# Orange-OpenSource/Cool-Chic

Hardware: AMD Instinct MI355X
Metric: decoded Mpixel/s (higher is better)
Workload: dtype int64+f64 entropy / f32 synthesis; 1 GPU; kodak24; frames_on_rank0=24, frame=512x768 RGB 8-bit, HOP decoder

## Files before the change

### cool_chic_amd/csrc/ccd_entropy_pipe.hip

```cpp
#include <hip/hip_runtime.h>
#include <type_traits>

#include "ccd_device.hpp"
#include "ccd_kernels.hpp"
#include "ccd_laplace.hpp"

namespace ccd {

#if defined(CCD_PIPE_PROFILE) && CCD_PIPE_PROFILE >= 3
#define PROF_T() __builtin_amdgcn_s_memtime()
#define PROF_ADD(var, t0) var += __builtin_amdgcn_s_memtime() - (t0)
#define PROF_SUB(var, t0) var -= __builtin_amdgcn_s_memtime() - (t0)
#else
#define PROF_T() 0ull
#define PROF_ADD(var, t0) (void)(t0)
#define PROF_SUB(var, t0) (void)(t0)
#endif
#if defined(CCD_PIPE_PROFILE) && CCD_PIPE_PROFILE == 2 && defined(CCD_PIPE_TRACE)
#define LPROF_T(cond) __builtin_amdgcn_s_memtime()
#elif defined(CCD_PIPE_PROFILE) && CCD_PIPE_PROFILE == 2
#define LPROF_T(cond) ((cond) ? __builtin_amdgcn_s_memtime() : 0ull)
#else
#define LPROF_T(cond) 0ull
#endif
#if defined(CCD_PIPE_TRACE)
constexpr int kTraceTasks = 512;
constexpr uint32_t kTraceLdsBytes = kTraceTasks * 32u;
__device__ unsigned int g_trace[kTraceTasks * 8];
__device__ unsigned int g_trace_cfg[2];
#endif

#ifndef CCD_T8
#define CCD_T8 25
#endif
#ifndef CCD_T4
#define CCD_T4 9
#endif
#ifndef CCD_PIPE_THREADS
#define CCD_PIPE_THREADS 512
#endif
constexpr int kPipeThreads = CCD_PIPE_THREADS;
constexpr int kPipeWaves = kPipeThreads / 64;
constexpr int kProducers = kPipeWaves - 1;
constexpr int kRows = 128;
constexpr int kSlots = 16;
constexpr int kMaxNV = 8;
constexpr int kRingRows = 512;
constexpr int kNarrowMaxScale = kScaleOffset;
constexpr int kIfceFastIn = 12;
constexpr unsigned kSpinLimit = 1u << 27;

struct alignas(16) RowMeta {
    double rcp[kRows + 2];
    int32_t mu_idx[kRows + 2];
    int32_t top[kRows + 2];
    uint32_t cell[kRows + 2];
    uint32_t goff[kRows + 2];
};
static_assert(offsetof(RowMeta, cell) - offsetof(RowMeta, top) == 520 && offsetof(RowMeta, goff) - offsetof(RowMeta, top) == 1040,
              "the decoder's asm region reads cell / goff at these immediate offsets from a top symbol's address");

extern __shared__ __attribute__((aligned(16))) unsigned char ccd_pipe_smem[];
template <typename T>
__device__ __forceinline__ T* smem_at(uint32_t off) { return reinterpret_cast<T*>(ccd_pipe_smem + off); }
template <typename T>
struct LdsRef {
    uint32_t off;
    __device__ __forceinline__ operator T*() const { return reinterpret_cast<T*>(ccd_pipe_smem + off); }
    __device__ __forceinline__ LdsRef& operator=(T* p) {
        off = static_cast<uint32_t>(reinterpret_cast<unsigned char*>(const_cast<typename std::remove_const<T>::type*>(p)) - ccd_pipe_smem);
        return *this;
    }
};

struct PipeLayout { uint32_t ring, w, b, act, a, tab, meta, rcp, exp, ready, consumed, abort, end; int n_w_hidden; };
__host__ __device__ constexpr PipeLayout pipe_layout(int dim, int n_layers, int in_pad, int ring_rows, int mf_tabs) {
    PipeLayout L{};
    L.ring = 0;
    L.w = static_cast<uint32_t>(ring_rows) * 64u;
    L.n_w_hidden = (n_layers - 1) * dim * in_pad;
    const int n_w_total = L.n_w_hidden + 4 * in_pad;
    L.b = L.w + static_cast<uint32_t>((n_w_total + 3) & ~3) * 4u;
    const int n_b_total = (n_layers - 1) * dim + 4;
    L.act = L.b + static_cast<uint32_t>((n_b_total + 1) & ~1) * 8u;
    L.a = L.act + static_cast<uint32_t>(kProducers * ((mf_tabs ? 16 : 8) * in_pad + 4)) * 4u;
    L.tab = L.a + static_cast<uint32_t>(mf_tabs) * 1024u;
    L.meta = L.tab + static_cast<uint32_t>(kRows + 1) * 64u * 8u;
    L.rcp = L.meta + static_cast<uint32_t>(sizeof(RowMeta));
    L.exp = L.rcp + static_cast<uint32_t>(kNumScale + 1) * 8u;
    L.ready = L.exp + static_cast<uint32_t>(1 << CCD_EXP_LOG) * 8u;
    L.consumed = L.ready + static_cast<uint32_t>(kSlots) * 4u;
    L.abort = L.consumed + 8u;
    L.end = (L.ready + static_cast<uint32_t>(kSlots + 8) * 4u + 15u) & ~15u;
    return L;
}

struct ShapeDyn { static constexpr bool fixed = false; static constexpr int dim = 0, n_layers = 0, n_sp = 0; };
template <int DIM, int NL, int NSP>
struct ShapeFix { static constexpr bool fixed = true; static constexpr int dim = DIM, n_layers = NL, n_sp = NSP; };
using ShapeHop = ShapeFix<20, 3, 14>;

__host__ __device__ constexpr int feat_stride(int n_if) { return n_if > 0 ? n_if : 1; }

struct PipeCtx {
    const EntropyParams* P;
    LdsRef<uint2> s_tab;
    LdsRef<RowMeta> s_meta;
    LdsRef<const double> s_rcp;
    LdsRef<const double> s_exp;
    LdsRef<int32_t> s_w;
    LdsRef<int64_t> s_b;
    LdsRef<int32_t> s_act;
    LdsRef<uint32_t> s_a;
    LdsRef<int8_t> s_ring;
    LdsRef<uint32_t> s_ready;
    LdsRef<uint32_t> s_consumed;
    LdsRef<uint32_t> s_abort;
// ... 668 lines not shown
            const uint32_t l_lo = static_cast<uint32_t>(__builtin_amdgcn_readlane(p_lo, k));
            const uint32_t l_hi = static_cast<uint32_t>(__builtin_amdgcn_readlane(p_hi, k));
            const uint32_t psel = static_cast<uint32_t>(__builtin_amdgcn_readlane(cur.y, k));
            uint64_t nd = rc_dist - ((static_cast<uint64_t>(l_hi) << 32) | l_lo);
            uint64_t nr = static_cast<uint64_t>(sc_lo) * psel + (static_cast<uint64_t>(sc_hi * psel) << 32);
            if (nr == 0) {
                S.n_search += 1;
                const uint64_t scale = rc_range >> kRcPrecision;
                if ((rc_dist >> kRcPrecision) >= scale) {
                    lds_write_release(C.s_abort, static_cast<uint32_t>(-CCD_ERR_INVALID_DATA));
                    ok = false;
                    break;
                }
                const double mu = -64.0 + static_cast<double>(meta.mu_idx[row0 + pi]) * (1.0 / 256.0);
                const double rcp = meta.rcp[row0 + pi];
                const uint32_t f0 = window_left(mu, rcp, kAcLo + lane, C.s_exp);
                const uint32_t f1 = window_left(mu, rcp, kAcLo + 64 + lane, C.s_exp);
                const unsigned long long m0 = __ballot(scale * f0 <= rc_dist), m1 = __ballot(scale * f1 <= rc_dist);
                const int sidx = __popcll(m0) + __popcll(m1) - 1;
                const uint32_t left = uni(static_cast<uint32_t>(__shfl(sidx < 64 ? f0 : f1, sidx & 63)));
                uint32_t right = uni(static_cast<uint32_t>(__shfl(sidx + 1 < 64 ? f0 : f1, (sidx + 1) & 63)));
                if (sidx == kAlphabet - 1) right = 1u << kRcPrecision;
                nd = rc_dist - scale * left;
                nr = scale * static_cast<uint64_t>(right - left);
                k = uni(1 - ((sidx + kAcLo) - meta.top[row0 + pi]));
            }
            if (static_cast<uint32_t>(nr >> 32) == 0) {
                nr <<= 32;
                nd = (nd << 32) | static_cast<uint32_t>(__builtin_amdgcn_readlane(wbuf, (word_pos - wbase) & 63));
                ++word_pos;
                if (word_pos - wbase == 64) { wbase = word_pos; wbuf = (wbase + lane < n_words) ? words_g[wbase + lane] : 0u; }
            }
            rc_dist = uni(nd); rc_range = uni(nr);
            asm volatile("s_mov_b32 m0, %2\n\tv_writelane_b32 %0, %1, m0" : "+v"(raw) : "s"(k), "s"(pi));
            ++i;
            mode = 1;
        }
    }
    S.dist = rc_dist; S.range = rc_range; S.word_pos = word_pos; S.wbase = wbase; S.wbuf = wbuf;
    S.n_spins += n_spins;
    S.n_part_batches += n_part;
    return seq;
}

__device__ __forceinline__ int64_t dot4(int4 x, int4 w) {
    return static_cast<int64_t>(x.x) * w.x + static_cast<int64_t>(x.y) * w.y + static_cast<int64_t>(x.z) * w.z +
           static_cast<int64_t>(x.w) * w.w;
}

__device__ __forceinline__ void mad64(int64_t& acc, int32_t x, int32_t w) {
    acc += static_cast<int64_t>(x) * static_cast<int64_t>(w);
    asm("" : "+v"(acc));
}
#define CCD_MAD4(ACC, X, Wv, NCH)                                                   \
    _Pragma("unroll") for (int g_ = 0; g_ < (NCH); ++g_) mad64(ACC[g_], (X).x, Wv[g_].x); \
    _Pragma("unroll") for (int g_ = 0; g_ < (NCH); ++g_) mad64(ACC[g_], (X).y, Wv[g_].y); \
    _Pragma("unroll") for (int g_ = 0; g_ < (NCH); ++g_) mad64(ACC[g_], (X).z, Wv[g_].z); \
    _Pragma("unroll") for (int g_ = 0; g_ < (NCH); ++g_) mad64(ACC[g_], (X).w, Wv[g_].w);
#define CCD_MAD4_PAIR(ACC, ACC2, X, Wv)                                             \
    mad64(ACC[0], (X).x, Wv[0].x); mad64(ACC2, (X).y, Wv[0].y); mad64(ACC[0], (X).z, Wv[0].z); mad64(ACC2, (X).w, Wv[0].w);


typedef int i32x4 __attribute__((ext_vector_type(4)));
constexpr int kMfLayer1 = 8;
constexpr int kMfHidden = 10;
constexpr int kMfOut = 5;
__host__ __device__ constexpr int mf_tables(int n_layers) { return kMfLayer1 + (n_layers - 2) * kMfHidden + kMfOut; }

__device__ __forceinline__ uint32_t mf_byte(int32_t w, int j) {
    const uint32_t d = (static_cast<uint32_t>(w) + 0x00808080u) ^ 0x00808080u;
    return (j < 0 || j > 2) ? 0u : ((d >> (8 * j)) & 0xffu);
}
__device__ __forceinline__ int mf_slot_input(bool first, int g, int beta, int n_sp, int n_if, int dim, int* limb) {
    if (first) {
        if (beta < 8) { *limb = 0; const int k = g + 4 * beta; return k < n_sp ? k : -1; }
        if (beta < 12) { *limb = (beta - 8) & 1; const int f = g + 4 * ((beta - 8) >> 1); return f < n_if ? n_sp + f : -1; }
        return -1;
    }
    if (beta >= 15) return -1;
    const int a = beta / 3;
    *limb = beta - 3 * a;
    const int k = a < 4 ? 4 * g + a : 16 + g;
    return k < dim ? k : -1;
}
__device__ __forceinline__ i32x4 mf_pack15(const int32_t (&a)[5]) {
    uint32_t d[5];
#pragma unroll
    for (int i = 0; i < 5; ++i) d[i] = ((static_cast<uint32_t>(a[i]) + 0x00808080u) ^ 0x00808080u) & 0x00ffffffu;
    i32x4 r;
    r[0] = static_cast<int>(d[0] | (d[1] << 24));
    r[1] = static_cast<int>((d[1] >> 8) | (d[2] << 16));
    r[2] = static_cast<int>((d[2] >> 16) | (d[3] << 8));
    r[3] = static_cast<int>(d[4]);
    return r;
}
__device__ __forceinline__ int64_t mf_comb4(const i32x4 (&c)[4], int r, int64_t bias) {
    const int32_t lo = c[0][r] + (c[1][r] << 8), hi = c[2][r] + (c[3][r] << 8);
    return bias + (static_cast<int64_t>(lo) << 16) + (static_cast<int64_t>(hi) << 32);
}
__device__ __forceinline__ int64_t mf_comb5(const i32x4 (&c)[5], int r, int64_t bias) {
    const int32_t lo = c[0][r] + (c[1][r] << 8), mid = c[2][r] + (c[3][r] << 8);
    return bias + lo + (static_cast<int64_t>(mid) << 16) + (static_cast<int64_t>(c[4][r]) << 32);
}

__device__ void mf_build_tables(const PipeCtx& C, int in_pad, uint32_t* s_a_words, int tid) {
    const int dim = C.dim, n_layers = C.n_layers, n_sp = C.n_sp, n_if = C.n_if;
    const int n_tab = mf_tables(n_layers);
    for (int e = tid; e < n_tab * 256; e += kPipeThreads) {
        const int idx = e >> 8, ln = (e >> 2) & 63, dw = e & 3, m = ln & 15, g = ln >> 4;
        int layer, tile, s;
        if (idx < kMfLayer1) { layer = 0; tile = idx >> 2; s = idx & 3; }
        else {
            const int j = idx - kMfLayer1, hl = j / kMfHidden;
// ... 216 lines not shown
        it.x0 = mv ? it.W - 10u : nx; it.y0 += mv; it.moved = mv; --it.left;
        it.n = min(it.H - it.y0, ((it.x0 * 0xcccdu) >> 19) + 1u);
    };
    while (n_steps_total - it.left < seg_end && it.next()) {
        const uint32_t seg_n = seg_body ? uni(seg.n_pix) : it.n;
        const uint32_t seg_pix0 = pix0;
        const uint32_t nb = (seg_n + kBpx - 1) >> kBpxShift;
        const uint32_t n_tasks = (seg_n + kTaskPix - 1) >> kTaskShift;
        const uint32_t seq0 = seq;
        uint32_t t_first = static_cast<uint32_t>(pw) - phase;
        t_first += static_cast<int32_t>(t_first) < 0 ? kProducers : 0;
        {
            for (uint32_t task = t_first; task < n_tasks; task += kProducers) {
                const uint32_t j = task >> kHalvesShift;
                const int half = static_cast<int>(task & (kHalves - 1));
                seq = seq0 + j;
                const int slot = static_cast<int>(seq & (kNSlots - 1));
                const int i0 = static_cast<int>(task << kTaskShift);
                const int cnt = min(kTaskPix, static_cast<int>(seg_n) - i0);
                while (seg_pix0 + static_cast<uint32_t>(i0) >= pix0 + it.n) walk_on();
                const uint32_t ia = seg_pix0 + static_cast<uint32_t>(i0) - pix0;
                const uint32_t n_a = min(static_cast<uint32_t>(cnt), it.n - ia);
                const uint32_t bx1 = it.x0 + 1u, b_moved = bx1 == static_cast<uint32_t>(W) ? 1u : 0u;
                const uint32_t bx0 = b_moved ? static_cast<uint32_t>(W) - 10u : bx1, by0 = it.y0 + b_moved;
                const bool in_b = static_cast<uint32_t>(px) >= n_a;
                const int ii = in_b ? px - static_cast<int>(n_a) : static_cast<int>(ia) + px;
                const int y = static_cast<int>(in_b ? by0 : it.y0) + ii, x = static_cast<int>(in_b ? bx0 : it.x0) - 10 * ii;
                const uint32_t dy1 = it.moved, dy2 = it.moved + prev_moved;
                const uint32_t prev_n = pix0 - prev_pix0, prev2_n = prev_pix0 - prev2_pix0;
                uint32_t f_raw[NOUT];
                bool f_has[NOUT];
                if constexpr (!MF) {
                    const int fo = (y >> 1) * fw + (x >> 1);
#pragma unroll
                    for (int t = 0; t < NOUT; ++t) {
                        const int k = q + kLpp * t;
                        f_has[t] = fin > 0 && px < cnt && k >= n_sp && k < dim;
                        f_raw[t] = reinterpret_cast<glb_ptr<const uint16_t>>(ifce_feat)[f_has[t] ? fo * fstride + (k - n_sp) : 0];
                    }
                } else {
#pragma unroll
                    for (int t = 0; t < NOUT; ++t) { f_raw[t] = 0; f_has[t] = false; }
                }
                unsigned long long bad_lanes = 0ull;
                const uint32_t need_slot = seq >= static_cast<uint32_t>(kNSlots) ? seq - kNSlots + 1 : 0;
                const bool ends_in_b = n_a < static_cast<uint32_t>(cnt);
                const uint32_t last1 = ends_in_b ? static_cast<uint32_t>(cnt) - n_a : ia + static_cast<uint32_t>(cnt);
                const uint32_t need_px = ends_in_b ? pix0 + min(last1 + b_moved, it.n) : prev_pix0 + min(last1 + dy1, prev_n);
                const uint32_t need_early_px = ends_in_b ? prev_pix0 + min(last1 + b_moved + dy1, prev_n)
                                                         : prev2_pix0 + min(last1 + dy2, prev2_n);
                unsigned long long lt_a = 0, lt_b = 0, lt_c = 0, lt_d = 0;
                (void)lt_a; (void)lt_b; (void)lt_c; (void)lt_d;
                unsigned narrow_mask = 0;
                unsigned long long wide_lanes = 0ull;
                RowMeta& meta = *C.s_meta;
                if constexpr (MF) {
                    const int n = px, g = q;
                    const bool live = n < cnt;
                    int32_t f0 = 0, f1 = 0;
                    if (live && fin > 0) {
                        const int fo = (y >> 1) * fw + (x >> 1);
                        if (g < n_if) f0 = ifce_feat[fo * fstride + g];
                        if (g + 4 < n_if) f1 = ifce_feat[fo * fstride + g + 4];
                    }
                    lt_a = LPROF_T(pw == 0);
#if defined(CCD_PIPE_PROFILE) && CCD_PIPE_PROFILE == 2
                    if (pw == 0 && lt_prev_end) prof[4] += lt_a - lt_prev_end;
#endif
                    {
                        const unsigned long long t0 = PROF_T();
                        if (!wait_ge2(C.s_consumed, need_slot, split ? need_early_px : need_px, C.s_abort)) return seq;
                        PROF_ADD(prof[0], t0);
                    }
                    lt_b = LPROF_T(pw == 0);
                    const unsigned long long t_g = PROF_T();
                    {
                        const int mi = (g == 0 && live) ? slot * kBpx + half * kTaskPix + n : kRows;
                        meta.cell[mi] = static_cast<uint32_t>(((y & ring_mask) << 6) | ((x + 10 * y) & 63));
                        meta.goff[mi] = static_cast<uint32_t>(y * W + x);
                    }
                    uint32_t w0 = 0, w1 = 0;
#pragma unroll
                    for (int t = 0; t < 8; ++t) {
                        if (4 * t < n_sp) {
                            const int k = g + 4 * t;
                            const int yy = y - (mf_dxy[t] >> 16), xx = x + static_cast<int16_t>(mf_dxy[t] & 0xffff);
                            const bool take = live && k < n_sp && yy >= 0 && xx >= 0 && xx < W && !(split && k == k_left);
                            const int cell = take ? (yy & ring_mask) * 64 + ((xx + 10 * yy) & 63) : 0;
                            int32_t v = C.s_ring[cell];
                            v = take ? v : 0;
                            if (t < 4) w0 |= static_cast<uint32_t>(v & 0xff) << (8 * t);
                            else w1 |= static_cast<uint32_t>(v & 0xff) << (8 * (t - 4));
                        }
                    }
                    const uint32_t d0 = (static_cast<uint32_t>(f0) + 0x8080u) ^ 0x8080u, d1 = (static_cast<uint32_t>(f1) + 0x8080u) ^ 0x8080u;
                    const i32x4 bop = {static_cast<int>(w0), static_cast<int>(w1), static_cast<int>((d0 & 0xffffu) | (d1 << 16)), 0};
                    PROF_ADD(prof[1], t_g);
                    const unsigned long long t_m = PROF_T();
                    const i32x4* sa = reinterpret_cast<const i32x4*>(static_cast<uint32_t*>(C.s_a)) + lane;
                    const i32x4 zero4 = {0, 0, 0, 0};
                    int64_t pre[5], st0, st1;
                    {
                        i32x4 c1[2][4];
#pragma unroll
                        for (int t = 0; t < 2; ++t)
#pragma unroll
// ... 180 lines not shown
#pragma unroll
                for (int v = 0; v < NV; ++v) xv[v] = act_row[v];
                PROF_ADD(prof[4], t_m);
                const unsigned long long t_s = PROF_T();
                int64_t so[2];
                const int qs = q < 2 ? q : 1;
                {
                    const int4* wr = reinterpret_cast<const int4*>(C.s_w + C.n_w_hidden + 2 * in_pad + qs * in_pad);
                    so[0] = C.s_b[(n_layers - 1) * dim + 2 + qs];
                    so[1] = 0;
                    int4 wv[NV];
#pragma unroll
                    for (int v = 0; v < NV; ++v) wv[v] = wr[v];
#pragma unroll
                    for (int v = 0; v < NV; ++v) {
                        const int4 w = wv[v];
                        mad64(so[0], xv[v].x, w.x); mad64(so[1], xv[v].y, w.y); mad64(so[0], xv[v].z, w.z); mad64(so[1], xv[v].w, w.w);
                    }
                }
                PROF_ADD(prof[5], t_s);
                const unsigned long long t_h = PROF_T();
                int64_t acc0[NOUT], acc0_b = 0;
                (void)acc0_b;
                int32_t wleft[NOUT], wleft_stab = 0;
                if (n_layers >= 2) {
                    const int32_t* wl = C.s_w;
                    const int64_t* bl = C.s_b;
                    const int4* wr[NOUT];
                    const int kl = split ? k_left : 0;
#pragma unroll
                    for (int t = 0; t < NOUT; ++t) {
                        const int oc = min(q + kLpp * t, dim - 1);
                        wr[t] = reinterpret_cast<const int4*>(wl + oc * in_pad);
                        acc0[t] = bl[oc];
                        wleft[t] = wl[oc * in_pad + kl];
                    }
                    wleft_stab = C.s_w[C.n_w_hidden + 2 * in_pad + qs * in_pad + kl];
                    int4 w[NOUT], wn[NOUT];
#pragma unroll
                    for (int t = 0; t < NOUT; ++t) w[t] = wr[t][0];
#pragma unroll
                    for (int v = 0; v < NV; ++v) {
                        if (v + 1 < NV) {
#pragma unroll
                            for (int t = 0; t < NOUT; ++t) wn[t] = wr[t][v + 1];
                        }
                        if constexpr (NOUT == 1) { CCD_MAD4_PAIR(acc0, acc0_b, xv[v], w) } else { CCD_MAD4(acc0, xv[v], w, NOUT) }
#pragma unroll
                        for (int t = 0; t < NOUT; ++t) w[t] = wn[t];
                    }
                    if constexpr (NOUT == 1) acc0[0] += acc0_b;
                }
                int32_t xleft = 0;
                lt_c = LPROF_T(pw == 0);
                if (split) {
                    const unsigned long long t0 = PROF_T();
                    const uint32_t want = uni(need_px);
                    const uint32_t cell = static_cast<uint32_t>((y & ring_mask) * 64 + ((x - 1 + 10 * y) & 63));
                    uint32_t seen_v;
                    int32_t r;
                    asm volatile("ds_read_b32 %0, %2 offset:4\n\tds_read_i8 %1, %3\n\ts_waitcnt lgkmcnt(0)"
                                 : "=&v"(seen_v), "=&v"(r) : "v"(C.s_consumed.off), "v"(C.s_ring.off + cell) : "memory");
                    if (__builtin_expect(static_cast<int32_t>(uni(seen_v) - want) < 0, 0)) {
                        unsigned spins = 0;
                        do {
                            if ((++spins & 1023u) == 0) {
                                if (lds_load_acquire(C.s_abort) != 0) return seq;
                                if (spins > kSpinLimit) { lds_write_release(C.s_abort, static_cast<uint32_t>(-CCD_ERR_HIP)); return seq; }
                            }
                            asm volatile("ds_read_b32 %0, %2 offset:4\n\tds_read_i8 %1, %3\n\ts_waitcnt lgkmcnt(0)"
                                         : "=&v"(seen_v), "=&v"(r) : "v"(C.s_consumed.off), "v"(C.s_ring.off + cell) : "memory");
                        } while (static_cast<int32_t>(uni(seen_v) - want) < 0);
                    }
                    PROF_ADD(prof[0], t0);
                    PROF_SUB(prof[2], t0);
                    PROF_SUB(prof[6], t0);
                    xleft = (px < cnt && x >= 1) ? r << 16 : 0;
                }
                lt_d = LPROF_T(pw == 0);
                __builtin_amdgcn_s_setprio(1);
                mad64(so[0], xleft, wleft_stab);
                const int64_t stab = so[0] + so[1];
                if (n_layers >= 2) {
#pragma unroll
                    for (int t = 0; t < NOUT; ++t) {
                        mad64(acc0[t], xleft, wleft[t]);
                        const int o = q + kLpp * t;
                        const int64_t a = acc0[t] < 0 ? 0 : acc0[t];
                        int32_t* const dst = o < in_pad ? act + px * in_pad + o : act_dummy;
                        *dst = o < dim ? static_cast<int32_t>(a >> 16) : 0;
                    }
#pragma unroll
                    for (int v = 0; v < NV; ++v) xv[v] = act_row[v];
                }
                for (int l = 1; l < n_layers - 1; ++l) {
                    const int32_t* wl = C.s_w + l * dim * in_pad;
                    const int64_t* bl = C.s_b + l * dim;
                    int64_t acc[NOUT], acc_b = 0;
                    (void)acc_b;
                    const int4* wr[NOUT];
#pragma unroll
                    for (int t = 0; t < NOUT; ++t) {
                        const int oc = min(q + kLpp * t, dim - 1);
                        wr[t] = reinterpret_cast<const int4*>(wl + oc * in_pad);
                        acc[t] = bl[oc];
                    }
                    int4 w[NOUT], wn[NOUT];
#pragma unroll
                    for (int t = 0; t < NOUT; ++t) w[t] = wr[t][0];
#pragma unroll
                    for (int v = 0; v < NV; ++v) {
                        if (v + 1 < NV) {
#pragma unroll
                            for (int t = 0; t < NOUT; ++t) wn[t] = wr[t][v + 1];
                        }
                        if constexpr (NOUT == 1) { CCD_MAD4_PAIR(acc, acc_b, xv[v], w) } else { CCD_MAD4(acc, xv[v], w, NOUT) }
#pragma unroll
                        for (int t = 0; t < NOUT; ++t) w[t] = wn[t];
                    }
                    if constexpr (NOUT == 1) acc[0] += acc_b;
#pragma unroll
                    for (int t = 0; t < NOUT; ++t) {
                        const int o = q + kLpp * t;
                        const int64_t a = acc[t] < 0 ? 0 : acc[t];
                        int32_t* const dst = o < in_pad ? act + px * in_pad + o : act_dummy;
                        *dst = o < dim ? static_cast<int32_t>(a >> 16) : 0;
                    }
#pragma unroll
                    for (int v = 0; v < NV; ++v) xv[v] = act_row[v];
                }
                PROF_ADD(prof[6], t_h);
                const unsigned long long t_o = PROF_T();
                const int mpx = slot * kBpx + half * kTaskPix + px;
                int32_t idx = 0;
                {
                    const int4* wr = reinterpret_cast<const int4*>(C.s_w + C.n_w_hidden + qs * in_pad);
                    int64_t ao[2] = {C.s_b[(n_layers - 1) * dim + qs] + stab, 0};
                    int4 wv[NV];
#pragma unroll
                    for (int v = 0; v < NV; ++v) wv[v] = wr[v];
#pragma unroll
                    for (int v = 0; v < NV; ++v) {
                        const int4 w = wv[v];
                        mad64(ao[0], xv[v].x, w.x); mad64(ao[1], xv[v].y, w.y); mad64(ao[0], xv[v].z, w.z); mad64(ao[1], xv[v].w, w.w);
                    }
                    const int64_t acc = ao[0] + ao[1];
                    const int64_t q8 = acc >> 24;
                    const int64_t off = q8 + (q == 0 ? kMuOffset : kScaleOffset);
                    const int64_t hi = q == 0 ? kNumMu - 1 : kNumScale - 1;
                    idx = static_cast<int32_t>(off < 0 ? 0 : (off > hi ? hi : off));
                    const bool live = px < cnt;
                    meta.mu_idx[live && q == 0 ? mpx : kRows] = idx;
                    meta.rcp[live && q == 1 ? mpx : kRows] = C.s_rcp[q == 1 ? idx : 0];
                }
                if (DYN && __builtin_expect(bad_lanes != 0ull, 0)) {
                    int n_redo = 0;
                    for (int p = 0; p < cnt; ++p) {
                        if (((bad_lanes >> (p * kLpp)) & ((1ull << kLpp) - 1ull)) == 0ull) continue;
                        ExactArgs A;
                        A.P = C.P; A.s_w = uni(C.s_w.off); A.s_b = uni(C.s_b.off); A.s_ring = uni(C.s_ring.off);
                        A.n_w_hidden = uni(C.n_w_hidden); A.dim = dim; A.n_layers = n_layers; A.n_sp = n_sp; A.in_pad = in_pad;
                        A.W = W; A.fin = fin; A.fw = fw; A.feat_plane = feat_plane; A.ring_mask = ring_mask; A.fstride = fstride;
                        asm volatile("" : "+s"(A.P), "+s"(A.s_w), "+s"(A.s_b), "+s"(A.s_ring), "+s"(A.n_w_hidden), "+s"(A.dim), "+s"(A.n_layers));
                        asm volatile("" : "+s"(A.n_sp), "+s"(A.W), "+s"(A.fin), "+s"(A.fw), "+s"(A.feat_plane), "+s"(A.ring_mask), "+s"(A.fstride));
                        const ExactOut r = exact_pixel(A, __builtin_amdgcn_readlane(y, MF ? p : p * kLpp), __builtin_amdgcn_readlane(x, MF ? p : p * kLpp));
                        if (px == p && q < 2) {
                            const int64_t off = ((q == 0 ? r.mu : r.ls) >> 24) + (q == 0 ? kMuOffset : kScaleOffset);
                            const int64_t hi = q == 0 ? kNumMu - 1 : kNumScale - 1;
                            idx = static_cast<int32_t>(off < 0 ? 0 : (off > hi ? hi : off));
                            if (q == 0) {
                                meta.mu_idx[mpx] = idx;
                            } else {
                                    meta.rcp[mpx] = C.s_rcp[idx];
                            }
                        }
                        ++n_redo;
                    }
                    if (lane == 0) atomicAdd(reinterpret_cast<int*>(P.status) + 39, n_redo);
                }
                wide_lanes = __ballot(q == 1 && px < cnt && idx > kNarrowMaxScale);
                PROF_ADD(prof[2], t_m);
                PROF_ADD(prof[7], t_o);
#if defined(CCD_PIPE_PROFILE) && CCD_PIPE_PROFILE >= 3
                prof[8] += 1;
#endif
                }
                const unsigned long long t_t = PROF_T();
                const int base = slot * kBpx + half * kTaskPix;
                uint2* tab = C.s_tab + static_cast<size_t>(base) * 64;
                if constexpr (!MF) {
                    for (int p4 = 0; p4 < cnt; p4 += 4) {
                        const int u = lane >> 4, e = lane & 15;
                        const int mine = p4 + u;
                        const bool valid = mine < cnt;
                        const int mi = base + (valid ? mine : p4);
                        const int mu_idx = meta.mu_idx[mi];
                        int top = ((mu_idx + 128) >> 8) - 64 + 6;
                        top = max(kAcLo + 13, min(kAcLo + kAlphabet - 1, top));
                        const double mu = -64.0 + static_cast<double>(mu_idx) * (1.0 / 256.0);
                        const int ssym = top - (e - 1);
                        uint32_t left = min(window_left(mu, meta.rcp[mi], ssym, C.s_exp), (1u << kRcPrecision) - 1u);
                        left = e == 15 ? 0u : left;
                        const uint32_t right = static_cast<uint32_t>(__builtin_amdgcn_update_dpp(0, static_cast<int>(left), 0x111, 0xf, 0xf, false));
                        uint2 ent;
                        ent.x = left;
                        const uint32_t to_full = (e == 1 && ssym == kAcLo + kAlphabet - 1) ? (1u << kRcPrecision) - right : 0u;
                        const uint32_t keep = (e == 0 || e == 15) ? 0u : ~0u;
                        ent.y = (right - left + to_full) & keep;
                        uint2* const row = valid ? tab + mine * 64 : C.s_tab + kRows * 64;
                        row[e] = ent;
                        meta.top[valid && e == 0 ? mi : kRows] = top;
                    }
                }
                unsigned rest = MF ? narrow_mask : 0u;
                while (rest) {
                    int pix[4];
                    int n_here = 0;
#pragma unroll
                    for (int u = 0; u < 4; ++u) {
                        pix[u] = rest ? __builtin_ctz(rest) : -1;
                        if (rest) { rest &= rest - 1; ++n_here; }
                    }
                    const int u = lane >> 4, e = lane & 15;
                    const int mine = u == 0 ? pix[0] : (u == 1 ? pix[1] : (u == 2 ? pix[2] : pix[3]));
                    const int mi = base + (mine < 0 ? pix[0] : mine);
                    const int mu_idx = meta.mu_idx[mi];
                    int top = ((mu_idx + 128) >> 8) - 64 + 6;
                    top = max(kAcLo + 13, min(kAcLo + kAlphabet - 1, top));
                    const double mu = -64.0 + static_cast<double>(mu_idx) * (1.0 / 256.0);
                    const int ssym = top - (e - 1);
                    uint32_t left = min(window_left(mu, meta.rcp[mi], ssym, C.s_exp), (1u << kRcPrecision) - 1u);
                    left = e == 15 ? 0u : left;
                    const uint32_t right = static_cast<uint32_t>(__builtin_amdgcn_update_dpp(0, static_cast<int>(left), 0x111, 0xf, 0xf, false));
                    uint2 ent;
                    ent.x = left;
                    ent.y = (e == 0 || e == 15) ? 0u : ((e == 1 && ssym == kAcLo + kAlphabet - 1) ? (1u << kRcPrecision) - left : right - left);
                    if (mine >= 0) {
                        tab[mine * 64 + e] = ent;
                        if (e == 0) meta.top[mi] = top;
                    }
                    if constexpr (MF) {
                        typedef unsigned int u32x4 __attribute__((ext_vector_type(4)));
                        const u32x4 z4 = {0u, 0u, 0u, 0u};
#pragma unroll
                        for (int j = 0; j < 2; ++j) {
                            const int t = lane + 64 * j;
                            const int ru = t >= 72 ? 3 : (t >= 48 ? 2 : (t >= 24 ? 1 : 0));
                            const int rp = ru == 0 ? pix[0] : (ru == 1 ? pix[1] : (ru == 2 ? pix[2] : pix[3]));
                            if (t < 96 && rp >= 0) *reinterpret_cast<u32x4*>(&tab[rp * 64 + 16 + 2 * (t - 24 * ru)]) = z4;
                        }
                    }
                    (void)n_here;
                }
                unsigned long long wide = MF ? static_cast<unsigned long long>(((1u << cnt) - 1u) & ~narrow_mask) : wide_lanes;
                while (wide) {
                    const int bit = __builtin_ctzll(wide);
                    wide &= wide - 1;
                    const int i = MF ? bit : bit / kLpp;
                    const int mi = base + i;
                    const int mu_idx = meta.mu_idx[mi];
                    int top = ((mu_idx + 128) >> 8) - 64 + 30;
                    top = max(kAcLo + 61, min(kAcLo + kAlphabet - 1, top));
                    const double mu = -64.0 + static_cast<double>(mu_idx) * (1.0 / 256.0);
                    const int ssym = top - (lane - 1);
                    uint32_t left = min(window_left(mu, meta.rcp[mi], ssym, C.s_exp), (1u << kRcPrecision) - 1u);
                    left = lane == 63 ? 0u : left;
                    const uint32_t right = __shfl_up(left, 1);
                    uint2 ent;
                    ent.x = left;
                    ent.y = (lane == 0 || lane == 63) ? 0u
                            : ((lane == 1 && ssym == kAcLo + kAlphabet - 1) ? (1u << kRcPrecision) - left : right - left);
                    tab[i * 64 + lane] = ent;
                    if (lane == 0) meta.top[mi] = top;
                }
                asm volatile("" ::: "memory");
                if (lane == 0) __hip_atomic_fetch_or(&C.s_ready[slot], 1u << half, __ATOMIC_RELAXED, __HIP_MEMORY_SCOPE_WORKGROUP);
                __builtin_amdgcn_s_setprio(0);
                asm volatile("" ::: "memory");
                PROF_ADD(prof[3], t_t);
#if defined(CCD_PIPE_PROFILE) && CCD_PIPE_PROFILE == 2
#if defined(CCD_PIPE_TRACE)
                {
                    const unsigned long long lt_e = __builtin_amdgcn_s_memtime();
                    const uint32_t gidx = seq0 * kHalves + task;
                    if (lane == 0 && static_cast<uint32_t>(W) == uni(g_trace_cfg[0]) && uni(g_trace_cfg[1]) - it.left < 64u) {
                        typedef unsigned int u32x4 __attribute__((ext_vector_type(4)));
                                                u32x4* r = reinterpret_cast<u32x4*>(ccd_pipe_smem + C.trace_off + (gidx % kTraceTasks) * 32u);
                        const u32x4 r0 = {(it.left << 12) | ((task & 15u) << 8) | (static_cast<uint32_t>(pw) << 4) | static_cast<uint32_t>(cnt), static_cast<uint32_t>(lt_a),
                                          static_cast<uint32_t>(lt_b), static_cast<uint32_t>(lt_c)};
                        const u32x4 r1 = {static_cast<uint32_t>(lt_d), static_cast<uint32_t>(lt_e), need_px - pix0, static_cast<uint32_t>(lt_a >> 32)};
                        r[0] = r0; r[1] = r1;
                    }
                }
#endif
                if (pw == 0) {
                    const unsigned long long lt_e = __builtin_amdgcn_s_memtime();
                    prof[0] += lt_b - lt_a; prof[1] += lt_c - lt_b; prof[2] += lt_d - lt_c; prof[3] += lt_e - lt_d; prof[8] += 1;
                    lt_prev_end = lt_e;
                }
#endif
            }
        }
        seq = seq0 + nb;
        phase = (phase + nb * kHalves) % kProducers;
        if (seg_body) {
            while (n_steps_total - it.left < seg_end) walk_on();
        }
        prev2_pix0 = prev_pix0;
        prev_pix0 = pix0;
        pix0 += it.n;
        prev_moved = it.moved;
    }
    return seq;
}

template <int NV, bool MF, bool DYN, class SH>
__global__ __launch_bounds__(kPipeThreads) void entropy_pipe_kernel(const EntropyParams* slots_desc) {
    const EntropyParams& P = slots_desc[blockIdx.x];
// ... 284 lines not shown
    }
#ifdef CCD_PIPE_PROFILE
    if (lane == 0 && wave < 2) {
        unsigned long long* o = reinterpret_cast<unsigned long long*>(P.status + 4) + wave * 5;
        o[0] = __builtin_amdgcn_s_memtime() - prof_total0;
        if (wave == 0) {
            o[1] = S.prof_wait; o[2] = S.prof_work; o[3] = prof_ifce; o[4] = prof_bar;
            P.status[38] = static_cast<int32_t>(S.n_spins);
        }
        else {
            o[1] = prof[0]; o[2] = prof[1]; o[3] = prof[2]; o[4] = prof[3];
            unsigned long long* e = reinterpret_cast<unsigned long long*>(P.status + 40);
            for (int i = 0; i < 5; ++i) e[i] = prof[4 + i];
        }
    }
#else
    (void)prof_total0; (void)prof_ifce; (void)prof_bar;
#endif
}

size_t entropy_pipe_lds_bytes(int dim, int n_layers, int ring_rows, int mfma) {
    size_t n = pipe_layout(dim, n_layers, (dim + 3) & ~3, ring_rows, mfma ? mf_tables(n_layers) : 0).end;
#if defined(CCD_PIPE_TRACE)
    n += kTraceLdsBytes;
#endif
    return n;
}

int entropy_pipe_ring_rows(int max_grid_w) {
    const int need = max_grid_w / 10 + 6;
    if (need > kRingRows) return 0;
    int r = 64;
    while (r < need) r *= 2;
    return r;
}

bool entropy_pipe_supports(int dim, int n_layers, int operands_ok, int max_grid_w) {
    const int ring = entropy_pipe_ring_rows(max_grid_w);
    return operands_ok && dim <= 4 * kMaxNV && n_layers <= 8 && ring > 0 && entropy_pipe_lds_bytes(dim, n_layers, kRingRows, 0) <= 160 * 1024;
}

bool entropy_pipe_supports_mfma(int dim, int n_layers, int n_ifce_out, int narrow, int max_grid_w, long long max_abs_weight) {
    const int ring = entropy_pipe_ring_rows(max_grid_w);
    return narrow && ring > 0 && dim <= 20 && n_layers >= 2 && n_layers <= 8 && n_ifce_out <= 8 &&
           max_abs_weight < (1ll << 23) && entropy_pipe_lds_bytes(dim, n_layers, ring, 1) <= 160 * 1024;
}

__global__ void laplace_sweep_pipe_kernel(const float* scale_table, const double* rcp_table, int scale_first, int n_scales, uint32_t* out) {
    const int64_t n = static_cast<int64_t>(n_scales) * kNumMu * 127;
    for (int64_t i = static_cast<int64_t>(blockIdx.x) * blockDim.x + threadIdx.x; i < n; i += static_cast<int64_t>(gridDim.x) * blockDim.x) {
        const int s = static_cast<int>(i % 127) - 63;
        const int64_t r = i / 127;
        const int mu_idx = static_cast<int>(r % kNumMu), c = scale_first + static_cast<int>(r / kNumMu);
        const double mu = -64.0 + static_cast<double>(mu_idx) * (1.0 / 256.0);
        out[i] = window_left(mu, rcp_table[c], s, kExpTab);
    }
}
hipError_t launch_laplace_sweep_pipe(const float* scale_table, const double* rcp_table, int scale_first, int n_scales, uint32_t* out, hipStream_t stream) {
    hipLaunchKernelGGL(laplace_sweep_pipe_kernel, dim3(256 * 16), dim3(256), 0, stream, scale_table, rcp_table, scale_first, n_scales, out);
    return hipGetLastError();
}

template <int NV, bool MF, bool DYN, class SH = ShapeDyn>
static hipError_t launch_pipe_nv(const EntropyParams* d_slots, int n_slots, size_t lds_bytes, hipStream_t stream) {
    hipError_t e = hipFuncSetAttribute(reinterpret_cast<const void*>(entropy_pipe_kernel<NV, MF, DYN, SH>),
                                       hipFuncAttributeMaxDynamicSharedMemorySize, static_cast<int>(lds_bytes));
    if (e != hipSuccess) return e;
    hipLaunchKernelGGL((entropy_pipe_kernel<NV, MF, DYN, SH>), dim3(n_slots), dim3(kPipeThreads), lds_bytes, stream, d_slots);
    return hipGetLastError();
}

int entropy_pipe_fixed_shape(int dim, int n_layers, int n_spatial) {
    return (dim == ShapeHop::dim && n_layers == ShapeHop::n_layers && n_spatial == ShapeHop::n_sp) ? 1 : 0;
}

hipError_t launch_entropy_pipe(const EntropyParams* d_slots, int n_slots, int nv, int mfma, int dyn, int shape, size_t lds_bytes, hipStream_t stream) {
    if (n_slots <= 0) return hipSuccess;
    if (shape == 1 && !mfma && nv == 5)
        return dyn ? launch_pipe_nv<5, false, true, ShapeHop>(d_slots, n_slots, lds_bytes, stream)
                   : launch_pipe_nv<5, false, false, ShapeHop>(d_slots, n_slots, lds_bytes, stream);
    if (shape != 0) return hipErrorInvalidValue;
    if (mfma) {
        switch (nv) {
            case 1: return launch_pipe_nv<1, true, false>(d_slots, n_slots, lds_bytes, stream);
            case 2: return launch_pipe_nv<2, true, false>(d_slots, n_slots, lds_bytes, stream);
            case 3: return launch_pipe_nv<3, true, false>(d_slots, n_slots, lds_bytes, stream);
            case 4: return launch_pipe_nv<4, true, false>(d_slots, n_slots, lds_bytes, stream);
            case 5: return launch_pipe_nv<5, true, false>(d_slots, n_slots, lds_bytes, stream);
            default: return hipErrorInvalidValue;
        }
    }
    if (dyn) {
        switch (nv) {
            case 1: return launch_pipe_nv<1, false, true>(d_slots, n_slots, lds_bytes, stream);
            case 2: return launch_pipe_nv<2, false, true>(d_slots, n_slots, lds_bytes, stream);
            case 3: return launch_pipe_nv<3, false, true>(d_slots, n_slots, lds_bytes, stream);
            case 4: return launch_pipe_nv<4, false, true>(d_slots, n_slots, lds_bytes, stream);
            case 5: return launch_pipe_nv<5, false, true>(d_slots, n_slots, lds_bytes, stream);
            case 6: return launch_pipe_nv<6, false, true>(d_slots, n_slots, lds_bytes, stream);
            case 7: return launch_pipe_nv<7, false, true>(d_slots, n_slots, lds_bytes, stream);
            case 8: return launch_pipe_nv<8, false, true>(d_slots, n_slots, lds_bytes, stream);
            default: return hipErrorInvalidValue;
        }
    }
    switch (nv) {
        case 1: return launch_pipe_nv<1, false, false>(d_slots, n_slots, lds_bytes, stream);
        case 2: return launch_pipe_nv<2, false, false>(d_slots, n_slots, lds_bytes, stream);
        case 3: return launch_pipe_nv<3, false, false>(d_slots, n_slots, lds_bytes, stream);
// ... 21 lines not shown
```

### cool_chic_amd/csrc/ccd_laplace.hpp

```cpp
#pragma once

#include "ccd_device.hpp"

namespace ccd {

#ifndef CCD_EXP_LOG
#define CCD_EXP_LOG 7
#endif
#ifndef CCD_EXP_DEG
#define CCD_EXP_DEG 5
#endif
#ifndef CCD_EXP_INC
#define CCD_EXP_INC "ccd_exp_table.inc"
#endif
static __device__ const double kExpTab[1 << CCD_EXP_LOG] = {
#include CCD_EXP_INC
};
constexpr int kExpLog = CCD_EXP_LOG, kExpN = 1 << kExpLog;
__device__ __forceinline__ double exp_nonpos(double x, const double* tab ) {
    const double kd = rint(x * ldexp(0x1.71547652b82fep+0, kExpLog));
    double r = fma(kd, -ldexp(0x1.62e42fef00000p-1, -kExpLog), x);
    r = fma(kd, -ldexp(0x1.473de6af278edp-34, -kExpLog), r);
    const int ki = static_cast<int>(kd);
    const double t = tab[ki & (kExpN - 1)];
    const double r2 = r * r;
#if CCD_EXP_DEG == 5
    double p = fma(r, 8.333333333333333e-03, 4.1666666666666664e-02);
    p = fma(p, r, 1.6666666666666666e-01);
    p = fma(p, r, 0.5);
#elif CCD_EXP_DEG == 4
    double p = fma(r, 4.1666666666666664e-02, 1.6666666666666666e-01);
    p = fma(p, r, 0.5);
#elif CCD_EXP_DEG == 3
    double p = fma(r, 1.6666666666666666e-01, 0.5);
#else
    double p = 0.5;
#endif
    p = fma(p, r2, r);
    return ldexp(fma(t, p, t), (ki >> kExpLog) - 1);
}

__device__ __forceinline__ uint32_t window_left(double mu, double rcp, int s, const double* exp_tab) {
    const double x = static_cast<double>(s) - 0.5;
    const double d = x - mu;
    const double e = exp_nonpos(-fabs(d) * rcp, exp_tab);
    const double cdf = d <= 0.0 ? e : 1.0 - e;
    const uint32_t v = static_cast<uint32_t>(16777088.0 * cdf) + static_cast<uint32_t>(s - kAcLo);
    return s <= kAcLo ? 0u : (s > kAcLo + kAlphabet - 1 ? (1u << kRcPrecision) : v);
}

}
```

Baseline: 259.3 Mpixel/s.

## Precompute LDS window addresses and use integer-scaled Laplace distance in entropy pipe

```diff
diff --git a/cool_chic_amd/csrc/ccd_entropy_pipe.hip b/cool_chic_amd/csrc/ccd_entropy_pipe.hip
--- a/cool_chic_amd/csrc/ccd_entropy_pipe.hip
+++ b/cool_chic_amd/csrc/ccd_entropy_pipe.hip
@@ -63,6 +63,13 @@
 extern __shared__ __attribute__((aligned(16))) unsigned char ccd_pipe_smem[];
 template <typename T>
 __device__ __forceinline__ T* smem_at(uint32_t off) { return reinterpret_cast<T*>(ccd_pipe_smem + off); }
+__device__ __forceinline__ uint32_t lds_addr(const void* p) {
+    return static_cast<uint32_t>(reinterpret_cast<uintptr_t>((__attribute__((address_space(3))) const char*)p));
+}
+template <typename T>
+__device__ __forceinline__ __attribute__((address_space(3))) T* lds_at(uint32_t addr) {
+    return reinterpret_cast<__attribute__((address_space(3))) T*>(static_cast<uintptr_t>(addr));
+}
 template <typename T>
 struct LdsRef {
     uint32_t off;
@@ -837,6 +844,9 @@
     acc += static_cast<int64_t>(x) * static_cast<int64_t>(w);
     asm("" : "+v"(acc));
 }
+__device__ __forceinline__ int32_t relu_q16(int64_t a) {
+    return static_cast<int32_t>(a >> 16) & ~static_cast<int32_t>(a >> 63);
+}
 #define CCD_MAD4(ACC, X, Wv, NCH)                                                   \
     _Pragma("unroll") for (int g_ = 0; g_ < (NCH); ++g_) mad64(ACC[g_], (X).x, Wv[g_].x); \
     _Pragma("unroll") for (int g_ = 0; g_ < (NCH); ++g_) mad64(ACC[g_], (X).y, Wv[g_].y); \
@@ -844,6 +854,19 @@
     _Pragma("unroll") for (int g_ = 0; g_ < (NCH); ++g_) mad64(ACC[g_], (X).w, Wv[g_].w);
 #define CCD_MAD4_PAIR(ACC, ACC2, X, Wv)                                             \
     mad64(ACC[0], (X).x, Wv[0].x); mad64(ACC2, (X).y, Wv[0].y); mad64(ACC[0], (X).z, Wv[0].z); mad64(ACC2, (X).w, Wv[0].w);
+__device__ __forceinline__ void mad64_seq(int64_t& acc, int32_t x, int32_t w) {
+    mad64(acc, x, w);
+    __builtin_amdgcn_sched_barrier(0);
+}
+#define CCD_MAD4_SEQ(ACC, X, Wv, NCH)                                               \
+    _Pragma("unroll") for (int g_ = 0; g_ < (NCH); ++g_) mad64_seq(ACC[g_], (X).x, Wv[g_].x); \
+    _Pragma("unroll") for (int g_ = 0; g_ < (NCH); ++g_) mad64_seq(ACC[g_], (X).y, Wv[g_].y); \
+    _Pragma("unroll") for (int g_ = 0; g_ < (NCH); ++g_) mad64_seq(ACC[g_], (X).z, Wv[g_].z); \
+    _Pragma("unroll") for (int g_ = 0; g_ < (NCH); ++g_) mad64_seq(ACC[g_], (X).w, Wv[g_].w);
+#define CCD_MAD4_PAIR_SEQ(ACC, ACC2, X, Wv)                                         \
+    mad64_seq(ACC[0], (X).x, Wv[0].x); mad64_seq(ACC2, (X).y, Wv[0].y); mad64_seq(ACC[0], (X).z, Wv[0].z); mad64_seq(ACC2, (X).w, Wv[0].w);
+#define CCD_MAD4_QUAD_SEQ(A4, X, W4)                                                \
+    mad64_seq(A4[0], (X).x, (W4).x); mad64_seq(A4[1], (X).y, (W4).y); mad64_seq(A4[2], (X).z, (W4).z); mad64_seq(A4[3], (X).w, (W4).w);
 
 
 typedef int i32x4 __attribute__((ext_vector_type(4)));
@@ -1166,6 +1189,10 @@
                 unsigned long long lt_a = 0, lt_b = 0, lt_c = 0, lt_d = 0;
                 (void)lt_a; (void)lt_b; (void)lt_c; (void)lt_d;
                 unsigned narrow_mask = 0;
+                constexpr int kPasses = (kTaskPix + 3) / 4;
+                uint32_t win_mu[kPasses] = {}, win_rcp[kPasses] = {}, win_ent[kPasses] = {}, win_top[kPasses] = {};
+                uint32_t win_left_m = 0, win_keep_m = 0, win_e0 = 0, win_e1 = 0;
+                (void)win_mu; (void)win_rcp; (void)win_ent; (void)win_top; (void)win_left_m; (void)win_keep_m; (void)win_e0; (void)win_e1;
                 unsigned long long wide_lanes = 0ull;
                 RowMeta& meta = *C.s_meta;
                 if constexpr (MF) {
@@ -1452,6 +1479,28 @@
                     if constexpr (NOUT == 1) acc0[0] += acc0_b;
                 }
                 int32_t xleft = 0;
+                const int mpx = slot * kBpx + half * kTaskPix + px;
+                uint32_t mu_dst = lds_addr(&meta.mu_idx[px < cnt && q == 0 ? mpx : kRows]);
+                uint32_t rcp_dst = lds_addr(&meta.rcp[px < cnt && q == 1 ? mpx : kRows]);
+                int32_t rcp_lanes = q == 1 ? -1 : 0, wide_above = px < cnt && q == 1 ? kNarrowMaxScale : 0x7fffffff;
+                asm volatile("" : "+v"(mu_dst), "+v"(rcp_dst), "+v"(rcp_lanes), "+v"(wide_above));
+#pragma unroll
+                for (int k = 0; k < kPasses; ++k) {
+                    const int u = lane >> 4, e = lane & 15;
+                    const int mine = 4 * k + u;
+                    const bool valid = mine < cnt;
+                    const int mi = slot * kBpx + half * kTaskPix + (valid ? mine : 4 * k);
+                    win_mu[k] = lds_addr(&meta.mu_idx[mi]);
+                    win_rcp[k] = lds_addr(&meta.rcp[mi]);
+                    win_ent[k] = lds_addr(&C.s_tab[static_cast<size_t>(valid ? mi : kRows) * 64 + e]);
+                    win_top[k] = lds_addr(&meta.top[valid && e == 0 ? mi : kRows]);
+                    asm volatile("" : "+v"(win_mu[k]), "+v"(win_rcp[k]), "+v"(win_ent[k]), "+v"(win_top[k]));
+                }
+                win_left_m = (lane & 15) == 15 ? 0u : ~0u;
+                win_keep_m = ((lane & 15) == 0 || (lane & 15) == 15) ? 0u : ~0u;
+                win_e0 = (lane & 15) == 0 ? (1u << kRcPrecision) - 1u : 0u;
+                win_e1 = (lane & 15) == 1 ? 1u : 0u;
+                asm volatile("" : "+v"(win_left_m), "+v"(win_keep_m), "+v"(win_e0), "+v"(win_e1));
                 lt_c = LPROF_T(pw == 0);
                 if (split) {
                     const unsigned long long t0 = PROF_T();
@@ -1486,9 +1535,8 @@
                     for (int t = 0; t < NOUT; ++t) {
                         mad64(acc0[t], xleft, wleft[t]);
                         const int o = q + kLpp * t;
-                        const int64_t a = acc0[t] < 0 ? 0 : acc0[t];
-                        int32_t* const dst = o < in_pad ? act + px * in_pad + o : act_dummy;
-                        *dst = o < dim ? static_cast<int32_t>(a >> 16) : 0;
+                        int32_t* const dst = o < dim ? act + px * in_pad + o : act_dummy;
+                        *dst = relu_q16(acc0[t]);
                     }
 #pragma unroll
                     for (int v = 0; v < NV; ++v) xv[v] = act_row[v];
@@ -1514,7 +1562,7 @@
 #pragma unroll
                             for (int t = 0; t < NOUT; ++t) wn[t] = wr[t][v + 1];
                         }
-                        if constexpr (NOUT == 1) { CCD_MAD4_PAIR(acc, acc_b, xv[v], w) } else { CCD_MAD4(acc, xv[v], w, NOUT) }
+                        if constexpr (NOUT == 1) { CCD_MAD4_PAIR_SEQ(acc, acc_b, xv[v], w) } else { CCD_MAD4_SEQ(acc, xv[v], w, NOUT) }
 #pragma unroll
                         for (int t = 0; t < NOUT; ++t) w[t] = wn[t];
                     }
@@ -1522,36 +1570,30 @@
 #pragma unroll
                     for (int t = 0; t < NOUT; ++t) {
                         const int o = q + kLpp * t;
-                        const int64_t a = acc[t] < 0 ? 0 : acc[t];
-                        int32_t* const dst = o < in_pad ? act + px * in_pad + o : act_dummy;
-                        *dst = o < dim ? static_cast<int32_t>(a >> 16) : 0;
+                        int32_t* const dst = o < dim ? act + px * in_pad + o : act_dummy;
+                        *dst = relu_q16(acc[t]);
                     }
 #pragma unroll
                     for (int v = 0; v < NV; ++v) xv[v] = act_row[v];
                 }
                 PROF_ADD(prof[6], t_h);
                 const unsigned long long t_o = PROF_T();
-                const int mpx = slot * kBpx + half * kTaskPix + px;
                 int32_t idx = 0;
                 {
                     const int4* wr = reinterpret_cast<const int4*>(C.s_w + C.n_w_hidden + qs * in_pad);
-                    int64_t ao[2] = {C.s_b[(n_layers - 1) * dim + qs] + stab, 0};
+                    int64_t ao[4] = {C.s_b[(n_layers - 1) * dim + qs] + stab, 0, 0, 0};
                     int4 wv[NV];
 #pragma unroll
                     for (int v = 0; v < NV; ++v) wv[v] = wr[v];
 #pragma unroll
-                    for (int v = 0; v < NV; ++v) {
-                        const int4 w = wv[v];
-                        mad64(ao[0], xv[v].x, w.x); mad64(ao[1], xv[v].y, w.y); mad64(ao[0], xv[v].z, w.z); mad64(ao[1], xv[v].w, w.w);
-                    }
-                    const int64_t acc = ao[0] + ao[1];
+                    for (int v = 0; v < NV; ++v) { CCD_MAD4_QUAD_SEQ(ao, xv[v], wv[v]) }
+                    const int64_t acc = (ao[0] + ao[1]) + (ao[2] + ao[3]);
                     const int64_t q8 = acc >> 24;
                     const int64_t off = q8 + (q == 0 ? kMuOffset : kScaleOffset);
                     const int64_t hi = q == 0 ? kNumMu - 1 : kNumScale - 1;
                     idx = static_cast<int32_t>(off < 0 ? 0 : (off > hi ? hi : off));
-                    const bool live = px < cnt;
-                    meta.mu_idx[live && q == 0 ? mpx : kRows] = idx;
-                    meta.rcp[live && q == 1 ? mpx : kRows] = C.s_rcp[q == 1 ? idx : 0];
+                    *lds_at<int32_t>(mu_dst) = idx;
+                    *lds_at<double>(rcp_dst) = C.s_rcp[idx & rcp_lanes];
                 }
                 if (DYN && __builtin_expect(bad_lanes != 0ull, 0)) {
                     int n_redo = 0;
@@ -1578,7 +1620,7 @@
                     }
                     if (lane == 0) atomicAdd(reinterpret_cast<int*>(P.status) + 39, n_redo);
                 }
-                wide_lanes = __ballot(q == 1 && px < cnt && idx > kNarrowMaxScale);
+                wide_lanes = __ballot(idx > wide_above);
                 PROF_ADD(prof[2], t_m);
                 PROF_ADD(prof[7], t_o);
 #if defined(CCD_PIPE_PROFILE) && CCD_PIPE_PROFILE >= 3
@@ -1589,27 +1631,28 @@
                 const int base = slot * kBpx + half * kTaskPix;
                 uint2* tab = C.s_tab + static_cast<size_t>(base) * 64;
                 if constexpr (!MF) {
-                    for (int p4 = 0; p4 < cnt; p4 += 4) {
-                        const int u = lane >> 4, e = lane & 15;
-                        const int mine = p4 + u;
-                        const bool valid = mine < cnt;
-                        const int mi = base + (valid ? mine : p4);
-                        const int mu_idx = meta.mu_idx[mi];
+#pragma unroll
+                    for (int k = 0; k < kPasses; ++k) {
+                        if (k > 0 && 4 * k >= cnt) break;
+                        const int e = lane & 15;
+                        const int mu_idx = *lds_at<int32_t>(win_mu[k]);
+                        const double rcp256 = window_rcp256(*lds_at<double>(win_rcp[k]));
                         int top = ((mu_idx + 128) >> 8) - 64 + 6;
                         top = max(kAcLo + 13, min(kAcLo + kAlphabet - 1, top));
-                        const double mu = -64.0 + static_cast<double>(mu_idx) * (1.0 / 256.0);
                         const int ssym = top - (e - 1);
-                        uint32_t left = min(window_left(mu, meta.rcp[mi], ssym, C.s_exp), (1u << kRcPrecision) - 1u);
-                        left = e == 15 ? 0u : left;
+                        const uint32_t lo_m = static_cast<uint32_t>((kAcLo - ssym) >> 31) & win_left_m;
+                        const bool at_top = top == kAcLo + kAlphabet - 1;
+                        const uint32_t hi_f = at_top ? win_e0 : 0u, to_full = at_top ? win_e1 : 0u;
+                        uint32_t left = window_cum_d256(window_d256(mu_idx, ssym), rcp256, C.s_exp) + static_cast<uint32_t>(ssym - kAcLo);
+                        left = (min(left, (1u << kRcPrecision) - 1u) | hi_f) & lo_m;
                         const uint32_t right = static_cast<uint32_t>(__builtin_amdgcn_update_dpp(0, static_cast<int>(left), 0x111, 0xf, 0xf, false));
                         uint2 ent;
                         ent.x = left;
-                        const uint32_t to_full = (e == 1 && ssym == kAcLo + kAlphabet - 1) ? (1u << kRcPrecision) - right : 0u;
-                        const uint32_t keep = (e == 0 || e == 15) ? 0u : ~0u;
-                        ent.y = (right - left + to_full) & keep;
-                        uint2* const row = valid ? tab + mine * 64 : C.s_tab + kRows * 64;
-                        row[e] = ent;
-                        meta.top[valid && e == 0 ? mi : kRows] = top;
+                        ent.y = (right - left + to_full) & win_keep_m;
+                        typedef unsigned int u32x2 __attribute__((ext_vector_type(2)));
+                        const u32x2 ent2 = {ent.x, ent.y};
+                        *lds_at<u32x2>(win_ent[k]) = ent2;
+                        *lds_at<int32_t>(win_top[k]) = top;
                     }
                 }
                 unsigned rest = MF ? narrow_mask : 0u;
@@ -1661,9 +1704,8 @@
                     const int mu_idx = meta.mu_idx[mi];
                     int top = ((mu_idx + 128) >> 8) - 64 + 30;
                     top = max(kAcLo + 61, min(kAcLo + kAlphabet - 1, top));
-                    const double mu = -64.0 + static_cast<double>(mu_idx) * (1.0 / 256.0);
                     const int ssym = top - (lane - 1);
-                    uint32_t left = min(window_left(mu, meta.rcp[mi], ssym, C.s_exp), (1u << kRcPrecision) - 1u);
+                    uint32_t left = min(window_left_d256(window_d256(mu_idx, ssym), window_rcp256(meta.rcp[mi]), ssym, C.s_exp), (1u << kRcPrecision) - 1u);
                     left = lane == 63 ? 0u : left;
                     const uint32_t right = __shfl_up(left, 1);
                     uint2 ent;
@@ -2054,8 +2096,7 @@
         const int s = static_cast<int>(i % 127) - 63;
         const int64_t r = i / 127;
         const int mu_idx = static_cast<int>(r % kNumMu), c = scale_first + static_cast<int>(r / kNumMu);
-        const double mu = -64.0 + static_cast<double>(mu_idx) * (1.0 / 256.0);
-        out[i] = window_left(mu, rcp_table[c], s, kExpTab);
+        out[i] = window_left_d256(window_d256(mu_idx, s), window_rcp256(rcp_table[c]), s, kExpTab);
     }
 }
 hipError_t launch_laplace_sweep_pipe(const float* scale_table, const double* rcp_table, int scale_first, int n_scales, uint32_t* out, hipStream_t stream) {
diff --git a/cool_chic_amd/csrc/ccd_laplace.hpp b/cool_chic_amd/csrc/ccd_laplace.hpp
--- a/cool_chic_amd/csrc/ccd_laplace.hpp
+++ b/cool_chic_amd/csrc/ccd_laplace.hpp
@@ -49,4 +49,16 @@
     return s <= kAcLo ? 0u : (s > kAcLo + kAlphabet - 1 ? (1u << kRcPrecision) : v);
 }
 
+__device__ __forceinline__ int window_d256(int mu_idx, int s) { return 256 * s + (256 * 64 - 128) - mu_idx; }
+__device__ __forceinline__ double window_rcp256(double rcp) { return ldexp(rcp, -8); }
+__device__ __forceinline__ uint32_t window_cum_d256(int d256, double rcp256, const double* exp_tab) {
+    const double e = exp_nonpos(-fabs(static_cast<double>(d256)) * rcp256, exp_tab);
+    const double cdf = d256 <= 0 ? e : 1.0 - e;
+    return static_cast<uint32_t>(16777088.0 * cdf);
 }
+__device__ __forceinline__ uint32_t window_left_d256(int d256, double rcp256, int s, const double* exp_tab) {
+    const uint32_t v = window_cum_d256(d256, rcp256, exp_tab) + static_cast<uint32_t>(s - kAcLo);
+    return s <= kAcLo ? 0u : (s > kAcLo + kAlphabet - 1 ? (1u << kRcPrecision) : v);
+}
+
+}
```

After: 264.3 Mpixel/s, median of 6. 1.02x the previous value.
